# tlangin/MDQTPlasmaSims

Hardware: AMD Instinct MI355X
Metric: particle-steps/sec (MD+QT) at N=3.5k and N=1M; 1/2/4/8-GPU scaling (higher is better)
Workload: dtype f64

## Files before the change

### mdqtplasmasims_amd/csrc/mdqt_engine.cpp

```cpp

#include <math.h>
#include <stdarg.h>
#include <stdlib.h>

#include <algorithm>
#include <thread>

#include "mdqt_ctx.hpp"
#include "mdqt_init_sample.hpp"

using namespace mdqt;

namespace {

thread_local std::string g_err;

struct cx { double re, im; };
inline cx cx_make(double r, double i) { return {r, i}; }
inline cx cx_mul(cx a, cx b) { return {a.re * b.re - a.im * b.im, a.re * b.im + a.im * b.re}; }
inline cx cx_add(cx a, cx b) { return {a.re + b.re, a.im + b.im}; }
inline cx cx_sub(cx a, cx b) { return {a.re - b.re, a.im - b.im}; }
inline cx cx_conj(cx a) { return {a.re, -a.im}; }


// ... 232 lines not shown
        else if (k == 4 || k == 5) e1 = 1.;
        else if (k == 6 || k == 7) e1 = 1. - q.kRat;
        else if (k == 8 || k == 9) e1 = -(1. + q.kRat);
        else if (k >= 10) e1 = q.kRat - 1.;
        f.mi0[k] = -(h * e0);
        f.mi1[k] = -(h * e1);
    }
    f.dms[8] = -(h * q.a8);  f.dmc[8] = h * q.a8;
    f.dms[9] = -(h * q.a11); f.dmc[9] = h * q.a11;
    f.dms[5] = h * q.a8;     f.dmc[5] = h * q.a8;
    f.dms[4] = h * q.a11;    f.dmc[4] = h * q.a11;
    const double kS = q.kickS * q.dtQ * q.gamToE, kD = q.kickD * q.dtQ * q.gamToE;
    struct KW { int row, col, g; double sgn, scale; };
    const KW kws[12] = {{1, 2, 0, 1., kS},  {0, 3, 2, 1., kS},  {1, 4, 4, -1., kS}, {0, 5, 5, -1., kS},
                        {8, 5, 8, 1., kD},  {9, 4, 11, 1., kD}, {10, 3, 14, 1., kD}, {11, 2, 17, 1., kD},
                        {6, 5, 6, -1., kD}, {7, 4, 9, -1., kD}, {8, 3, 12, -1., kD}, {9, 2, 15, -1., kD}};
    for (const KW& w : kws)
        for (int j = 0; j < 3; ++j)
            if (kFastCol[w.col][j] == w.row) f.kw[j][w.col] = -(w.sgn * (w.scale * gs[w.g]));
    f.cphi = 2. * (1. + q.kRat) * q.gamToE;
    if (p->qt_model != 0) build_pump_tables(p, q, f);
    f.dt2 = (0.5 * q.dtQ) * (0.5 * q.dtQ);
    for (int k = 0; k < 4; ++k) q.hdPh[k] = f.hdp[2 + k];
    FastTab& fl = s->ftabL;
    fl = f;
    {
        double kw = 0.;
        for (int j = 0; j < 3; ++j)
            for (int k = 0; k < 16; ++k) kw += fabs(f.kw[j][k]);
        q.kickmax = fmax(fabs(q.vKick), fabs(q.vKickDP)) + 16. * kw;
    }
    q.im01 = 1;
    for (int k = 0; k < 16; ++k)
        if (f.cre[0][k] != 0. || f.cre[1][k] != 0.) q.im01 = 0;
    if (p->qt_model == 0) {
        memset(&fl, 0, sizeof fl);
        fl.cphi = f.cphi; fl.dt2 = f.dt2;
        for (int l = 0; l < 16; ++l) {
            for (int j = 0; j < 3; ++j) fl.col[j][l] = l;
            const int k = state_of_lane0(l);
            if (k >= NS) continue;
            for (int j = 0; j < 3; ++j) {
                fl.cre[j][l] = f.cre[j][k]; fl.cim[j][l] = f.cim[j][k]; fl.kw[j][l] = f.kw[j][k];
            }
            fl.dms[l] = f.dms[k]; fl.dmc[l] = f.dmc[k]; fl.mre[l] = f.mre[k];
            fl.mi0[l] = f.mi0[k]; fl.mi1[l] = f.mi1[k]; fl.hdp[l] = f.hdp[k];
// ... 485 lines not shown
```

### mdqtplasmasims_amd/csrc/mdqt_ensemble_qt.hip

```cpp
#include "mdqt_ens_args.hpp"
#include "mdqt_qtfast.hpp"

namespace mdqt {

#define LANE_ENS_KERNELS(SUFFIX, ATTR, JUNI)                                                                        \
    template <bool DPPX, bool FAST>                                                                                 \
    __global__ __launch_bounds__(256) ATTR void k_substeps_lanes_r_ens##SUFFIX(const SubstepArgs* __restrict__ jobs, \
                                                                               const FastTab* __restrict__ tab) {   \
        const SubstepArgs& a = jobs[blockIdx.y];                                                                    \
        if ((int)blockIdx.x * kLaneIons >= a.n) return;                                                             \
        lane_substeps<DPPX, FAST, false, false, false, false, JUNI>(a, tab, blockIdx.x);                            \
    }                                                                                                               \
    template <bool DPPX, bool EDZ, bool NORN = false>                                                               \
    __global__ __launch_bounds__(256) ATTR void k_substeps_lanes_im_ens##SUFFIX(const SubstepArgs* __restrict__ jobs, \
                                                                                const FastTab* __restrict__ tab) {  \
        const SubstepArgs& a = jobs[blockIdx.y];                                                                    \
        if ((int)blockIdx.x * kLaneIons >= a.n) return;                                                             \
        lane_substeps<DPPX, true, false, true, EDZ, NORN, JUNI>(a, tab, blockIdx.x);                                \
    }
LANE_ENS_KERNELS(, , true)
LANE_ENS_KERNELS(_w3, __attribute__((amdgpu_waves_per_eu(3, 3))), false)
#undef LANE_ENS_KERNELS

hipError_t launch_substeps_r_ens(const SubstepArgs* jobs, const SubstepArgs& a, int njobs, int max_n, const FastTab* tab,
                                 int wpe, hipStream_t s, hipEvent_t ev0, hipEvent_t ev1, int* instance) {
    if (njobs <= 0 || max_n <= 0 || a.nsub <= 0) return hipSuccess;
    if (!jobs || njobs > 65535 || a.nsub > MAXSUB || a.qc.model != 0 || a.arrive || a.U) return hipErrorInvalidValue;
    if (wpe != 0 && wpe != 3) return hipErrorInvalidValue;
    const dim3 gl((max_n + kLaneIons - 1) / kLaneIons, njobs), bl(kLaneWG);
    const FastTab* lt = tab + 1;
    const QTKernel inst = lane_qt_instance(a);
    switch (inst) {
    case QTK_LANES_IM_EDZ:
        if (wpe == 3) launch_timed(k_substeps_lanes_im_ens_w3<true, true, true>, gl, bl, s, ev0, ev1, jobs, lt);
        else launch_timed(k_substeps_lanes_im_ens<true, true, true>, gl, bl, s, ev0, ev1, jobs, lt);
        break;
    case QTK_LANES_IM_EDZ_RN: launch_timed(k_substeps_lanes_im_ens<true, true>, gl, bl, s, ev0, ev1, jobs, lt); break;
    case QTK_LANES_IM: launch_timed(k_substeps_lanes_im_ens<true, false>, gl, bl, s, ev0, ev1, jobs, lt); break;
    case QTK_LANES_R_FAST: launch_timed(k_substeps_lanes_r_ens<true, true>, gl, bl, s, ev0, ev1, jobs, lt); break;
    case QTK_LANES_R: launch_timed(k_substeps_lanes_r_ens<true, false>, gl, bl, s, ev0, ev1, jobs, lt); break;
    default: return hipErrorInvalidValue;
    }
    if (instance) *instance = inst;
    return hipGetLastError();
}

}
```

### mdqtplasmasims_amd/csrc/mdqt_ensemble_sweep_qt.hip

```cpp
#include "mdqt_ens_args.hpp"
#include "mdqt_qtfast.hpp"

namespace mdqt {

#define LANE_SWEEP_KERNELS(SUFFIX, ATTR, JUNI)                                                                         \
    template <bool DPPX, bool FAST>                                                                                    \
    __global__ __launch_bounds__(256) ATTR void k_substeps_lanes_r_sweep##SUFFIX(const SubstepArgs* __restrict__ jobs, \
                                                                                 const FastTab* __restrict__ tabs,     \
                                                                                 const int* __restrict__ point) {      \
        const SubstepArgs& a = jobs[blockIdx.y];                                                                       \
        if ((int)blockIdx.x * kLaneIons >= a.n) return;                                                                \
        lane_substeps<DPPX, FAST, false, false, false, false, JUNI>(a, tabs + point[blockIdx.y], blockIdx.x);          \
    }                                                                                                                  \
    template <bool DPPX, bool EDZ, bool NORN = false>                                                                  \
    __global__ __launch_bounds__(256) ATTR void k_substeps_lanes_im_sweep##SUFFIX(const SubstepArgs* __restrict__ jobs, \
                                                                                  const FastTab* __restrict__ tabs,    \
                                                                                  const int* __restrict__ point) {     \
        const SubstepArgs& a = jobs[blockIdx.y];                                                                       \
        if ((int)blockIdx.x * kLaneIons >= a.n) return;                                                                \
        lane_substeps<DPPX, true, false, true, EDZ, NORN, JUNI>(a, tabs + point[blockIdx.y], blockIdx.x);              \
    }
LANE_SWEEP_KERNELS(, , true)
LANE_SWEEP_KERNELS(_w3, __attribute__((amdgpu_waves_per_eu(3, 3))), false)
#undef LANE_SWEEP_KERNELS

hipError_t launch_substeps_r_sweep(const SubstepArgs* jobs, const SubstepArgs* h, int njobs, int max_n, const FastTab* tabs,
                                   const int* point, int wpe, hipStream_t s, hipEvent_t ev0, hipEvent_t ev1, int* instance,
                                   int* differs) {
    if (differs) *differs = -1;
    if (njobs <= 0 || max_n <= 0) return hipSuccess;
    if (!jobs || !h || !tabs || !point || njobs > 65535) return hipErrorInvalidValue;
    const SubstepArgs& a = h[0];
    if (a.nsub <= 0) return hipSuccess;
    if (a.nsub > MAXSUB || a.qc.model != 0 || a.arrive || a.U) return hipErrorInvalidValue;
    if (wpe != 0 && wpe != 3) return hipErrorInvalidValue;
    for (int k = 1; k < njobs; ++k)
        if (sweep_choice_differs(a, h[k])) {
            if (differs) *differs = k;
            return hipErrorInvalidValue;
        }
    const dim3 gl((max_n + kLaneIons - 1) / kLaneIons, njobs), bl(kLaneWG);
    const QTKernel inst = lane_qt_instance(a);
    switch (inst) {
    case QTK_LANES_IM_EDZ:
        if (wpe == 3) launch_timed(k_substeps_lanes_im_sweep_w3<true, true, true>, gl, bl, s, ev0, ev1, jobs, tabs, point);
        else launch_timed(k_substeps_lanes_im_sweep<true, true, true>, gl, bl, s, ev0, ev1, jobs, tabs, point);
        break;
    case QTK_LANES_IM_EDZ_RN: launch_timed(k_substeps_lanes_im_sweep<true, true>, gl, bl, s, ev0, ev1, jobs, tabs, point); break;
    case QTK_LANES_IM: launch_timed(k_substeps_lanes_im_sweep<true, false>, gl, bl, s, ev0, ev1, jobs, tabs, point); break;
    case QTK_LANES_R_FAST: launch_timed(k_substeps_lanes_r_sweep<true, true>, gl, bl, s, ev0, ev1, jobs, tabs, point); break;
    case QTK_LANES_R: launch_timed(k_substeps_lanes_r_sweep<true, false>, gl, bl, s, ev0, ev1, jobs, tabs, point); break;
    default: return hipErrorInvalidValue;
    }
    if (instance) *instance = inst;
    return hipGetLastError();
}

}
```

### mdqtplasmasims_amd/csrc/mdqt_internal.hpp

```cpp
#pragma once
#include <hip/hip_runtime.h>
#if defined(__HIP__)
#include <hip/hip_ext.h>
#include <type_traits>
#endif
#include <stdint.h>

namespace mdqt {

constexpr int NS = 12;
constexpr int NBINS = 2001;
constexpr int MAXSUB = 32;
constexpr int NSTATIC = 20;
constexpr double kKdeV2 = 1. / (2. * 0.002 * 0.002);
constexpr double kKdeSkip = 0.0773;
static_assert(kKdeV2 * kKdeSkip * kKdeSkip * (1. - 1e-12) >= 746.0, "KDE skip threshold must lie beyond exp's underflow");

constexpr int kStaticRC[NSTATIC][2] = {
    {0, 3}, {0, 5}, {1, 2}, {1, 4}, {2, 1}, {2, 9}, {2, 11}, {3, 0}, {3, 8}, {3, 10},
    {4, 1}, {4, 7}, {5, 0}, {5, 6}, {6, 5}, {7, 4}, {8, 3}, {9, 2}, {10, 3}, {11, 2}};

struct QTConst {
    double dtQ, gamToE;
    double h, dtHalf, invh;
    double pv2q;
    double kRat, r;
    double det, detDP;
    double kickS, kickD;
    double vKick, vKickDP;
    double pD;
    double dP[4];
    double hdP[4];
    double hdPh[4];
    double a8, a11;
    double Mre[NSTATIC], Mim[NSTATIC];
    double thS3, thS4;
    double thD[4][2];
    double gs[18];
    double kickmax;
    int renorm;
    int im01;
    int model;
    uint32_t seed, job;
};

struct LaneTab {
    int colA[16], colB[16], colC[16];
    int order[16], hasB[16], hasC[16];
    int dynB[16], dynC[16];
    double cAre[16], cAim[16], cBre[16], cBim[16], cCre[16], cCim[16];
    double dynScale[16];
    double gA[16], gB[16];
    double dP[16];
    double hd[16];
};

constexpr int NMODELS = 4;
constexpr int kModelStates[NMODELS] = {12, 7, 7, 5};
constexpr int kFastColM[NMODELS][NS][3] = {
    {{5, 12, 3}, {4, 12, 2}, {9, 11, 1}, {8, 10, 0}, {1, 7, 9}, {0, 6, 8},
     {12, 5, 12}, {12, 4, 12}, {3, 12, 5}, {2, 12, 4}, {12, 3, 12}, {12, 2, 12}},
    {{2, 4, 0}, {3, 5, 1}, {0, 2, 2}, {1, 3, 3}, {0, 4, 4}, {1, 5, 5},
     {6, 6, 6}, {7, 7, 7}, {8, 8, 8}, {9, 9, 9}, {10, 10, 10}, {11, 11, 11}},
    {{4, 0, 0}, {5, 1, 1}, {2, 2, 2}, {3, 3, 3}, {0, 4, 4}, {1, 5, 5},
     {6, 6, 6}, {7, 7, 7}, {8, 8, 8}, {9, 9, 9}, {10, 10, 10}, {11, 11, 11}},
    {{3, 0, 0}, {2, 1, 1}, {1, 2, 2}, {0, 3, 3}, {4, 4, 4}, {5, 5, 5},
     {6, 6, 6}, {7, 7, 7}, {8, 8, 8}, {9, 9, 9}, {10, 10, 10}, {11, 11, 11}}};
// ... 127 lines not shown
    else g(std::integral_constant<int, 0>{});
}
#endif

enum QTKernel : int {
    QTK_NONE = 0,
    QTK_LANES_IM_EDZ = 1,
    QTK_LANES_IM = 2,
    QTK_LANES_R_FAST = 3,
    QTK_LANES_R = 4,
    QTK_LANES_R_PUMP_FAST = 5,
    QTK_LANES_R_PUMP = 6,
    QTK_LANES_IM_EDZ_RN = 7,
    QTK_THREAD_R = 10,
    QTK_MD_STEP = 20,
    QTK_EXACT_LANES = 30,
    QTK_EXACT_THREAD = 40,
};
hipError_t launch_substeps(const SubstepArgs& a, const LaneTab* tab, int mode, int fast, hipStream_t s,
                           hipEvent_t ev0 = nullptr, hipEvent_t ev1 = nullptr, int* instance = nullptr);
hipError_t launch_substeps_r(const SubstepArgs& a, const FastTab* tab, int mode, hipStream_t s,
                             hipEvent_t ev0 = nullptr, hipEvent_t ev1 = nullptr,
                             int* instance = nullptr);
hipError_t launch_md_step(const N3Args& f, const SubstepArgs& a, const FastTab* tab, int variant, hipStream_t s,
                          hipEvent_t ev0 = nullptr, hipEvent_t ev1 = nullptr);

hipError_t launch_tag_spin_up(const double* psi, int n, int S, uint64_t gid0, uint64_t q, const QTConst& qc,
                              int* tags, hipStream_t s);
hipError_t launch_sum_vx(const double* V, int n, double* out, hipStream_t s, double* avg = nullptr, int N = 0);
hipError_t launch_output_pack(const double* V, const double* psi, int n, int S, int model, double* out,
                              hipStream_t s);
hipError_t launch_energy_sums(const double* V, int n, int S, const double* vxAvg,
                              const double* urow, double* out, hipStream_t s);
hipError_t launch_kde(const double* V, int n, int S, const double* vxAvg, double* Ppart,
                      int nchunk, double* Pout, hipStream_t s);

}
```

### mdqtplasmasims_amd/csrc/mdqt_options.cpp

```cpp

#include <math.h>
#include <stdlib.h>

#include "mdqt_ctx.hpp"

using namespace mdqt;

struct TierConst { const char *radius, *bound; int mdqt_ctx::*exp; int level; };
static const TierConst kTierConsts[] = {
    {"force_far_radius", "force_far_bound", &mdqt_ctx::far_exp, 1},
    {"force_mid_radius", "force_mid_bound", &mdqt_ctx::mid_exp, 5},
    {"force_vfar_radius", "force_vfar_bound", &mdqt_ctx::vfar_exp, 2},
    {"force_ufar_radius", "force_ufar_bound", &mdqt_ctx::ufar_exp, 3},
};
static double tier_const(const mdqt_ctx* s, int k, int level, double* bound) {
    *bound = 0.;
    const bool on = s->use_n3b && s->sort_mode != 0 && s->force_variant == 1 && !s->guard;
    return on ? tier_radius(s, k, level, bound) : s->L / 2.;
}

extern "C" double mdqt_get_const(const mdqt_ctx* s, const char* n) {
    if (!strcmp(n, "gamToEinsteinFreq")) return s->gamToE;
    if (!strcmp(n, "quantumTimestep")) return s->dtQ;
    if (!strcmp(n, "plasmaToQuantumTimestepRatio")) return s->ratio;
// ... 64 lines not shown
        tier_radii(s, a);
        return error_eps(s, a);
    }
    for (const TierConst& tc : kTierConsts) {
        const bool radius = !strcmp(n, tc.radius);
        if (!radius && strcmp(n, tc.bound)) continue;
        double bound;
        double r = tier_const(s, s->*tc.exp, tc.level, &bound);
        if (tc.level == 3) {
            if (r < s->L / 2. && s->L / 2. > 80. * s->lDeb) { r = s->L / 2.; bound = 0.; }
            double b32 = 0.;
            if (r < s->L / 2.) tier_radius(s, s->ufar_exp, 4, &b32);
            bound += b32;
        }
        return radius ? r : bound;
    }
    if (!strcmp(n, "force_ufar32_radius")) {
        double bound;
        const double r3 = mdqt_get_const(s, "force_ufar_radius");
        return r3 < s->L / 2. ? tier_radius(s, s->ufar_exp, 4, &bound) : s->L / 2.;
    }
    if (!strcmp(n, "fused_step")) return s->fused_opt;
    if (!strcmp(n, "qt_im01")) return s->qc.im01;
    if (!strcmp(n, "potential_n3")) return s->n3_potential;
    if (!strcmp(n, "potential_plan")) return s->pot_plan;
    if (!strcmp(n, "force_n3b_pairs")) return s->n3b_pairs;
    if (!strcmp(n, "md_step_fused")) return s->last_fused;
    if (!strcmp(n, "qt_kernel")) return s->last_qt_kernel;
    if (!strcmp(n, "qt_kernel_nseg")) return s->last_qt_nseg;
    if (!strcmp(n, "force_slots")) return s->nslots;
    if (!strcmp(n, "n3b_blocks")) return s->use_n3b ? s->n3b.Phi - s->n3b.Plo : 0;
    if (!strcmp(n, "n3b_block_count")) return s->use_n3b ? s->n3b.NB : 0;
    if (!strcmp(n, "slab_S")) return s->S;
    if (!strncmp(n, "gs", 2)) return s->gs[atoi(n + 2)];
    return NAN;
}

enum Invalidates {
    NOTHING,
    SETTLE,
    SETTLE_RESET,
    SETTLE_AUX,
};
struct Option {
    const char* name;
    int lo, hi;
// ... 6 lines not shown

static int set_force_scheme(mdqt_ctx* s, int value) {
    if (value == 2 && s->p.world_size != 1) return set_error("force_scheme 2 needs world_size 1");
    if (settle_forces(s)) return -1;
    s->scheme_opt = value;
    choose_segments(s);
    return ensure_aux(s);
}
static int set_expt_force_sig(mdqt_ctx* s, int value) {
    if (value && arrive_setup(s)) return -1;
    s->force_arrive = value ? s->dArrive : nullptr;
    return 0;
}
static int set_qt_im01(mdqt_ctx* s, int value) {
    if (value) {
        int ok = 1;
        for (int k = 0; k < 16; ++k)
            if (s->ftab.cre[0][k] != 0. || s->ftab.cre[1][k] != 0.) ok = 0;
        if (!ok) return set_error("qt_im01: the static coupling slots are not purely imaginary");
    }
    s->qc.im01 = value;
    return 0;
}
static int set_force_balance(mdqt_ctx* s, int value) {
    if (value != s->balance_opt) {
        if (settle_forces(s)) return -1;
        s->balance_opt = value;
        if (s->use_n3b) {
            const int W = s->p.world_size;
            n3b_set_range(s->n3b, (int)((long)s->p.rank * s->n3b.NB / W), (int)((long)(s->p.rank + 1) * s->n3b.NB / W));
            s->balanced = false;
            if (ensure_aux(s)) return -1;
        }
    }
    return 0;
}
static int set_qt_enabled(mdqt_ctx* s, int value) { s->p.qt_enabled = value; return 0; }
static int set_qt_math(mdqt_ctx* s, int value) {
    if (value != 2 && s->p.qt_model != 0) return set_error("the optical-pumping qt_models need qt_math 2");
    s->qt_math = value;
    return 0;
}

static const Option kOptions[] = {
    {"force_scheme", 0, 3, "force_scheme must be 0 (auto), 1 (rows), 2 (Newton-3 tiles) or 3 (Newton-3 blocks)",
     NOTHING, nullptr, set_force_scheme},
    {"expt_force_sig", 0, 1, "expt_force_sig must be 0 or 1", NOTHING, nullptr, set_expt_force_sig},
    {"potential_n3", 0, 1, "potential_n3 must be 0 or 1", NOTHING, &mdqt_ctx::n3_potential},
    {"force_n3b_pairs", 0, 1, "force_n3b_pairs must be 0 (8 waves, one I tile each) or 1 (4 waves, two each)",
     SETTLE, &mdqt_ctx::n3b_pairs},
    {"potential_plan", 0, 1, "potential_plan must be 0 (every pair to L/2) or 1 (the plan)", NOTHING, &mdqt_ctx::pot_plan},
    {"qt_im01", 0, 1, "qt_im01 must be 0 or 1", NOTHING, nullptr, set_qt_im01},
    {"fused_step", 0, 1, "fused_step must be 0 or 1", NOTHING, &mdqt_ctx::fused_opt},
    {"overlap", 0, 1, "overlap must be 0 or 1", NOTHING, &mdqt_ctx::overlap_opt},
    {"force_ufar_exp", 0, 300, "force_ufar_exp must be 0 (off) .. 300", SETTLE_RESET, &mdqt_ctx::ufar_exp, nullptr, form_measured},
    {"force_vfar_exp", 0, 300, "force_vfar_exp must be 0 (off) .. 300", SETTLE_RESET, &mdqt_ctx::vfar_exp, nullptr, form_measured},
    {"force_mid_exp", 0, 300, "force_mid_exp must be 0 (off) .. 300", SETTLE_RESET, &mdqt_ctx::mid_exp, nullptr, form_measured},
    {"force_far_exp", 0, 300, "force_far_exp must be 0 (off) .. 300", SETTLE_RESET, &mdqt_ctx::far_exp, nullptr, form_measured},
    {"force_tail_exp", 0, 300, "force_tail_exp must be 0 (exact) .. 300", SETTLE_RESET, &mdqt_ctx::tail_exp},
    {"force_form_mode", 0, 2, "force_form_mode must be 0 (a priori), 1 (measured) or 2 (measured, sharing an exact tail's eps)",
     SETTLE_RESET, &mdqt_ctx::form_mode},
    {"force_tail_mode", 0, 1, "force_tail_mode must be 0 (a priori) or 1 (measured)", SETTLE_RESET, &mdqt_ctx::tail_mode},
    {"force_balance", 0, 1, "force_balance must be 0 (equal block counts) or 1 (by work)", NOTHING, nullptr, set_force_balance},
    {"force_tile_split", 0, 2, "force_tile_split must be 0 (off), 1 (halves) or 2 (quarters)", SETTLE_AUX, &mdqt_ctx::split_opt},
    {"force_split_cus", 0, 65536, "force_split_cus must be 0 (the device's CU count) or a CU count",
     SETTLE_AUX, &mdqt_ctx::split_cus},
    {"force_reduce_mask", 0, 1, "force_reduce_mask must be 0 (every j-slot) or 1 (the written ones)",
     SETTLE, &mdqt_ctx::tmask_mode},
    {"force_ax1", 0, 1, "force_ax1 must be 0 (off) or 1 (where the skip radius reaches L/2)", SETTLE, &mdqt_ctx::ax1_mode},
    {"force_sort", 0, 2, "force_sort must be 0 (off), 1 (on) or 2 (sorted, no skipping)", SETTLE_AUX, &mdqt_ctx::sort_mode},
    {"qt_enabled", 0, 1, "qt_enabled must be 0 or 1", NOTHING, nullptr, set_qt_enabled},
    {"qt_math", 0, 2, "qt_math must be 0 (exact), 1 (FMA-contracted) or 2 (reassociated)", NOTHING, nullptr, set_qt_math},
    {"force_kernel", 0, 1, "force_kernel must be 0 (exact) or 1 (fast)", SETTLE_RESET, &mdqt_ctx::force_variant},
    {"init_threads", 0, 256, "init_threads must be in [0, 256]", NOTHING, &mdqt_ctx::init_threads},
    {"substep_kernel", 0, 2, "substep_kernel must be 0 (auto), 1 (thread/ion) or 2 (lanes/ion)", NOTHING, &mdqt_ctx::substep_mode},
// ... 127 lines not shown
```

### mdqtplasmasims_amd/csrc/mdqt_qtfast.hip

```cpp
#include "mdqt_qtfast.hpp"
#include "mdqt_pump_device.hpp"

namespace mdqt {

template <int MODEL>
__device__ __forceinline__ double sum_p(const double* Tp) {
    if constexpr (MODEL == 0) return ((Tp[0] + Tp[2]) + Tp[1]) + Tp[3];
    return (Tp[0] + Tp[1]) + (Tp[2] + Tp[3]);
}
template <int MODEL>
__device__ __forceinline__ double tree_lanes(const double* vs) {
    double v[16];
#pragma unroll
    for (int l = 0; l < 16; ++l) {
        const int st = MODEL == 0 ? state_of_lane0(l) : l;
        v[l] = st < NS ? vs[st] : 0.;
    }
    return tree16n(v);
}

template <int MODEL>
__global__ __launch_bounds__(256) void k_substeps_r(SubstepArgs a, const FastTab* __restrict__ tab) {
    constexpr const int(&COL)[NS][3] = kFastColM[MODEL];
    const int i = blockIdx.x * 256 + threadIdx.x;
// ... 181 lines not shown
    } else {
        if (variant == 1) launch_timed(k_md_step<false, 1>, gl, bl, s, ev0, ev1, f, a, lt);
        else launch_timed(k_md_step<false, 0>, gl, bl, s, ev0, ev1, f, a, lt);
    }
    return hipGetLastError();
}

#if defined(MDQT_EXPT_QTSTAMPS)
extern "C" int mdqt_expt_qt_stamps(unsigned long long* out, int nwaves) {
    return hipMemcpyFromSymbol(out, HIP_SYMBOL(g_qt_stamps), sizeof(unsigned long long) * 16 * nwaves) == hipSuccess ? 0 : -1;
}
#endif

hipError_t launch_substeps_r(const SubstepArgs& a, const FastTab* tab, int mode, hipStream_t s, hipEvent_t ev0,
                             hipEvent_t ev1, int* instance) {
    if (a.n <= 0 || a.nsub <= 0) return hipSuccess;
    if (a.nsub > MAXSUB) return hipErrorInvalidValue;
    if (mode == 0) mode = (a.n < kLaneKernelMaxIons) ? 2 : 1;
    if (a.qc.model < 0 || a.qc.model >= NMODELS) return hipErrorInvalidValue;
    const dim3 gl((a.n + kLaneIons - 1) / kLaneIons), bl(kLaneWG), gt((a.n + 255) / 256), b(256);
    int inst = QTK_THREAD_R + a.qc.model;
    if (mode == 2) {
        const FastTab* lt = tab + 1;
        switch (inst = lane_qt_instance(a)) {
        case QTK_LANES_IM_EDZ: launch_timed(k_substeps_lanes_im<true, true, true>, gl, bl, s, ev0, ev1, a, lt); break;
        case QTK_LANES_IM_EDZ_RN: launch_timed(k_substeps_lanes_im<true, true>, gl, bl, s, ev0, ev1, a, lt); break;
        case QTK_LANES_IM: launch_timed(k_substeps_lanes_im<true, false>, gl, bl, s, ev0, ev1, a, lt); break;
        case QTK_LANES_R_FAST: launch_timed(k_substeps_lanes_r<true, true>, gl, bl, s, ev0, ev1, a, lt); break;
        case QTK_LANES_R: launch_timed(k_substeps_lanes_r<true, false>, gl, bl, s, ev0, ev1, a, lt); break;
        case QTK_LANES_R_PUMP_FAST: launch_timed(k_substeps_lanes_r<false, true>, gl, bl, s, ev0, ev1, a, lt); break;
        case QTK_LANES_R_PUMP: launch_timed(k_substeps_lanes_r<false, false>, gl, bl, s, ev0, ev1, a, lt); break;
        default: return hipErrorInvalidValue;
        }
    }
    else if (a.qc.model == 0) launch_timed(k_substeps_r<0>, gt, b, s, ev0, ev1, a, tab);
    else if (a.qc.model == 1) launch_timed(k_substeps_r<1>, gt, b, s, ev0, ev1, a, tab);
    else if (a.qc.model == 2) launch_timed(k_substeps_r<2>, gt, b, s, ev0, ev1, a, tab);
    else launch_timed(k_substeps_r<3>, gt, b, s, ev0, ev1, a, tab);
    if (instance) *instance = inst;
    return hipGetLastError();
}

__global__ __launch_bounds__(256) void k_tag_spin_up(const double* __restrict__ psi, int n, int S, uint64_t gid0,
                                                     uint64_t q, QTConst qc, int* __restrict__ tags) {
    const int i = blockIdx.x * 256 + threadIdx.x;
    if (i >= n) return;
    tag_spin_up_ion(psi, i, S, gid0, q, qc, tags);
// ... 11 lines not shown
```

### mdqtplasmasims_amd/csrc/mdqt_qtfast.hpp

```cpp
#pragma once
#include "mdqt_internal.hpp"
#if defined(__HIP__)
#include "mdqt_device.hpp"
#include "mdqt_pairs.hpp"

#include <math.h>

#include <type_traits>

namespace mdqt {

constexpr int kLaneWG = 256;
static_assert(kLaneWG % 64 == 0 && kLaneWG >= 128, "whole waves; the first 128 threads stage the sincos table");
constexpr int kRows = 4;
constexpr int kLaneIons = kLaneWG / 64 * kRows;

__device__ __forceinline__ double rsq_nr(double x) { return rsq3(x); }
__device__ __forceinline__ double nrm2(cxd y) { return fma(y.re, y.re, y.im * y.im); }
__device__ __forceinline__ double rho_im_r(cxd a, cxd b) { return fma(a.im, b.re, -(a.re * b.im)); }

__device__ __forceinline__ cxd row_r(cxd md, cxd y, cxd c0, cxd y0, cxd c1, cxd y1, cxd c2, cxd y2) {
    double re = md.re * y.re, im = md.re * y.im;
    re = fma(-md.im, y.im, re);  im = fma(md.im, y.re, im);
    re = fma(c0.re, y0.re, re);  im = fma(c0.re, y0.im, im);
// ... 120 lines not shown
    double a = dpp<BCAST(0)>(T);
    a = fmac_bcast<3>(a, T, one);
    a = fmac_bcast<4>(a, T, one);
    return fmac_bcast<7>(a, T, one);
}

__device__ __forceinline__ void qt_store(double* p, double v) {
    __hip_atomic_store(p, v, __ATOMIC_RELAXED, __HIP_MEMORY_SCOPE_AGENT);
}

#if defined(MDQT_EXPT_QTSTAMPS)
__device__ unsigned long long g_qt_stamps[16 * 4096];
#define QT_STAMP(slot, v) (st_[slot] = (v))
#define QT_JCOUNT(c) (st_[7] += (__builtin_amdgcn_ballot_w64(c) != 0))
#else
#define QT_STAMP(slot, v) ((void)0)
#define QT_JCOUNT(c) ((void)0)
#endif

#if defined(MDQT_EXPT_MDSTAMPS)
__device__ unsigned long long g_md_stamps[4 * 4096];
#endif

template <bool DPPX, bool FAST, bool FUSED, bool IM01 = false, bool EDZ = false, bool NORN = false, bool JUNI = !FUSED>
__device__ __forceinline__ void lane_substeps(const SubstepArgs& a, const FastTab* __restrict__ tab, int blk) {
#if defined(MDQT_EXPT_QTSTAMPS)
    unsigned long long st_[16] = {};
#endif
    QT_STAMP(0, __builtin_amdgcn_s_memtime());
    QT_STAMP(4, __builtin_amdgcn_s_memrealtime());
    const int k = threadIdx.x & 15;
    const int grp = threadIdx.x >> 4;
    const int iraw = blk * (kLaneWG / 16) + grp;
    const bool store = iraw < a.n;
    const int i = store ? iraw : a.n - 1;
    const QTConst& qc = a.qc;
    const int S = a.S;
    const int st = DPPX ? state_of_lane0(k) : k;
    const int cy = DPPX ? 9 : 12, cz = DPPX ? 10 : 13;
    const int c = (k == cy) ? 1 : (k == cz) ? 2 : 0;
    const bool owner = (k == 0) || (k == cy) || (k == cz);
    const int base = threadIdx.x & ~15;
    const int l0 = base + tab->col[0][k], l1 = base + tab->col[1][k], l2 = base + tab->col[2][k];
    const cxd c0 = {tab->cre[0][k], tab->cim[0][k]}, c1 = {tab->cre[1][k], tab->cim[1][k]};
    const double c2re = tab->cre[2][k], c2im = tab->cim[2][k], dms = tab->dms[k], dmc = tab->dmc[k];
    const double mre = tab->mre[k], mi0 = tab->mi0[k], mi1 = tab->mi1[k], hdp = tab->hdp[k];
    const double kw0 = tab->kw[0][k], kw1 = tab->kw[1][k], kw2 = tab->kw[2][k];
    const double cphi = tab->cphi, DT2 = tab->dt2;
// ... 38 lines not shown
            slot_add(t);
        }
    };
    double t0[4][3];
    if (FAST) {
        if (!FUSED) slot_round(k, t0, false);
    } else if (nseg > 1) {
        if (!a.arrive) slot_partials(false);
    } else {
        f = a.F[(size_t)c * S + i];
    }
    QT_STAMP(9, __builtin_amdgcn_s_memtime());
    const double L = a.L, dt = qc.dtQ, DT = 0.5 * dt;
    double dtq_v = qc.dtQ, pv2q_v = qc.pv2q;
    asm volatile("" : "+v"(dtq_v), "+v"(pv2q_v));
    const uint64_t gid = a.gid0 + (uint64_t)i;
    const uint32_t movmask = a.movmask;
    __shared__ double edt[MAXSUB];
    const double edv = (threadIdx.x < MAXSUB && a.expdet_zero == 0 && (int)threadIdx.x < a.nsub)
                           ? a.expDet[threadIdx.x] : 0.;
    __shared__ double sct[128];
    const double sctv = threadIdx.x < 128 ? kSinCos64[threadIdx.x] : 0.;
    __shared__ double su[kLaneWG / 16][MAXSUB][2];
    if (FAST || a.do_qt) {
        if (a.U) {
            if (k == 0) { su[grp][0][0] = a.U[i]; su[grp][0][1] = a.U[(size_t)S + i]; }
        } else {
            for (int s = k; s < a.nsub; s += 16) {
                double x0, x1;
                philox_pair(qc, gid, a.q0 + (uint64_t)s, 0, x0, x1);
                su[grp][s][0] = x0;
                su[grp][s][1] = x1;
            }
        }
    }
    QT_STAMP(8, __builtin_amdgcn_s_memtime());
    if (!FAST && a.arrive) {
        if (threadIdx.x == 0) {
            int it = 0;
            const unsigned long long* cnt = a.arrive + (blk * (kLaneWG / 16)) / 64;
            while (__hip_atomic_load(cnt, __ATOMIC_ACQUIRE, __HIP_MEMORY_SCOPE_AGENT) < a.arrive_target) {
                for (int z = 0; z < a.arrive_sleep; ++z) __builtin_amdgcn_s_sleep(1);
                if (++it > (1 << 21)) { *a.spin_err = 1; break; }
            }
        }
        __syncthreads();
        __atomic_thread_fence(__ATOMIC_ACQUIRE);
        if (nseg > 1) slot_partials(true);
    }
// ... 9 lines not shown
        __syncthreads();
        __atomic_thread_fence(__ATOMIC_ACQUIRE);
#if defined(MDQT_EXPT_MDSTAMPS)
        if (threadIdx.x == 0 && blockIdx.x < 4096) g_md_stamps[4 * blockIdx.x + 2] = __builtin_amdgcn_s_memrealtime();
#endif
        slot_round(k, t0, true);
    }
    if (FAST) {
        slot_add(t0);
        for (int s0 = k + 64; s0 < nseg; s0 += 64) {
            double t[4][3];
            slot_round(s0, t, FUSED);
            slot_add(t);
        }
    }
    QT_STAMP(6, __builtin_amdgcn_s_memtime());
    if (FAST || nseg > 1) {
        const double fx = lane_tree16(qf[0]), fy = lane_tree16(qf[1]), fz = lane_tree16(qf[2]);
        f = c == 0 ? fx : c == 1 ? fy : fz;
        if (store && owner) qt_store(&a.F[(size_t)c * S + i], f);
    }
    if (threadIdx.x < MAXSUB) edt[threadIdx.x] = edv;
    if (threadIdx.x < 128) sct[threadIdx.x] = sctv;
    __syncthreads();
    __shared__ double2 xg[DPPX ? 1 : kLaneWG];
    auto exchange = [&](cxd y, cxd& y0, cxd& y1, cxd& y2) {
        if constexpr (DPPX) {
            y0 = {dpp<QP_XOR2>(y.re), dpp<QP_XOR2>(y.im)};
            y1 = {dpp<ROR(8)>(y.re), dpp<ROR(8)>(y.im)};
            y2 = {dpp<QP_XOR1>(y.re), dpp<QP_XOR1>(y.im)};
            return;
        }
        wave_sync();
        xg[threadIdx.x] = make_double2(y.re, y.im);
        wave_sync();
        const double2 t0 = xg[l0], t1 = xg[l1], t2 = xg[l2];
        y0 = {t0.x, t0.y}; y1 = {t1.x, t1.y}; y2 = {t2.x, t2.y};
    };
    auto drift = [&](double& pp, double& vv, int sub) {
        const bool moving = FAST || ((movmask >> sub) & 1u);
        pp = half_drift(pp, vv, f, moving, DT, DT2, L);
        vv = vv + dt * f;
        pp = half_drift(pp, vv, f, moving, DT, DT2, L);
    };
    QT_STAMP(1, __builtin_amdgcn_s_memtime());
    if (!FAST && !a.do_qt) {
// ... 87 lines not shown
                    (void)dummy;
                } else {
                    double x0, x1;
                    philox_pair(qc, gid, a.q0 + (uint64_t)s, k < 8 ? 1 : 2, x0, x1);
                    randDOrS = dpp<BCAST(0)>(x0);
                    randDir = dpp<BCAST(0)>(x1);
                    rand3 = dpp<BCAST(8)>(x0);
                }
                return (DPPX || qc.model == 0)
                           ? jump_target(qc, n3, n4, n5, n6, u2, randDOrS, randDir, rand3, jkick)
                           : jump_target_pump(qc, n3, n4, n5, n6, u2, randDOrS, randDir, rand3, jkick);
            };
            if constexpr (JUNI) {
            auto jump_substep = [&](auto tape) {
                const double kick_rk = rk_kick();
                const cxd w_rk = rk_stages();
                double kick_j;
                const int target = jump(tape, kick_j);
                w = {nojump ? w_rk.re : (st == target ? 1. : 0.), nojump ? w_rk.im : 0.};
                kick = nojump ? kick_rk : kick_j;
                tPart = nojump ? tPart : 0.;
                next_phase();
            };
            if (__builtin_expect(__builtin_amdgcn_ballot_w64(!nojump) == 0, 1)) {
                kick = rk_kick();
                next_phase();
                w = rk_stages();
            } else if (a.U) {
                jump_substep(std::true_type{});
            } else {
                jump_substep(std::false_type{});
            }
            } else if (nojump) {
                kick = rk_kick();
                next_phase();
                w = rk_stages();
            } else {
                tPart = 0;
                int target;
                if (a.U) target = jump(std::true_type{}, kick);
                else target = jump(std::false_type{}, kick);
                w = {st == target ? 1. : 0., 0.};
                next_phase();
            }
            if constexpr (decltype(chk)::value)
                if (!(fabs(phin) < 1048576.)) sincos(phin, &snn, &csn);
            if (!NORN && qc.renorm) w = [&] {
                const double r = rsq_nr(lane_norm16(nrm2(w), one));
                return cxd{w.re * r, w.im * r};
            }();
            v = vn;
            p = pn;
            u = un;
            sn = snn;
// ... 49 lines not shown

namespace mdqt {

inline QTKernel lane_qt_instance(const SubstepArgs& a) {
    const uint64_t all = (1ull << a.nsub) - 1;
    const bool allmove = a.do_step && a.do_qt && a.nseg >= 1 && !a.arrive && (a.movmask & all) == all;
    if (a.qc.model != 0) return allmove ? QTK_LANES_R_PUMP_FAST : QTK_LANES_R_PUMP;
    if (!allmove) return QTK_LANES_R;
    if (!a.qc.im01) return QTK_LANES_R_FAST;
    if (!a.expdet_zero) return QTK_LANES_IM;
    return a.qc.renorm ? QTK_LANES_IM_EDZ_RN : QTK_LANES_IM_EDZ;
}
inline const char* sweep_choice_differs(const SubstepArgs& a, const SubstepArgs& b) {
    if (a.nsub != b.nsub) return "nsub";
    if (a.do_step != b.do_step) return "do_step";
    if (a.do_qt != b.do_qt) return "do_qt";
    if (a.movmask != b.movmask) return "movmask (t > 0 per substep)";
    if (a.expdet_zero != b.expdet_zero) return "expdet_zero (fracOfSig == 0 against != 0)";
    if (a.qc.im01 != b.qc.im01) return "qt_im01";
    if (a.qc.renorm != b.qc.renorm) return "reNormalizewvFns";
    if (a.qc.model != b.qc.model) return "qt_model";
    if ((a.nseg >= 1) != (b.nseg >= 1)) return "nseg";
    if (!a.arrive != !b.arrive || !a.U != !b.U) return "arrive / U (another launch scheme)";
    return nullptr;
}

}
```

Measured before the change: 2.886 billion.

## Stage jump constants in LDS and optionally predraw jump random candidates

```diff
diff --git a/mdqtplasmasims_amd/csrc/mdqt_engine.cpp b/mdqtplasmasims_amd/csrc/mdqt_engine.cpp
--- a/mdqtplasmasims_amd/csrc/mdqt_engine.cpp
+++ b/mdqtplasmasims_amd/csrc/mdqt_engine.cpp
@@ -278,6 +278,7 @@
     if (p->qt_model != 0) build_pump_tables(p, q, f);
     f.dt2 = (0.5 * q.dtQ) * (0.5 * q.dtQ);
     for (int k = 0; k < 4; ++k) q.hdPh[k] = f.hdp[2 + k];
+    jump_predraw_setup(q, f.hdp, 1);
     FastTab& fl = s->ftabL;
     fl = f;
     {
diff --git a/mdqtplasmasims_amd/csrc/mdqt_ensemble_qt.hip b/mdqtplasmasims_amd/csrc/mdqt_ensemble_qt.hip
--- a/mdqtplasmasims_amd/csrc/mdqt_ensemble_qt.hip
+++ b/mdqtplasmasims_amd/csrc/mdqt_ensemble_qt.hip
@@ -3,23 +3,24 @@
 
 namespace mdqt {
 
-#define LANE_ENS_KERNELS(SUFFIX, ATTR, JUNI)                                                                        \
+#define LANE_ENS_KERNELS(SUFFIX, ATTR, JUNI, JPRE)                                                                    \
     template <bool DPPX, bool FAST>                                                                                 \
     __global__ __launch_bounds__(256) ATTR void k_substeps_lanes_r_ens##SUFFIX(const SubstepArgs* __restrict__ jobs, \
                                                                                const FastTab* __restrict__ tab) {   \
         const SubstepArgs& a = jobs[blockIdx.y];                                                                    \
         if ((int)blockIdx.x * kLaneIons >= a.n) return;                                                             \
-        lane_substeps<DPPX, FAST, false, false, false, false, JUNI>(a, tab, blockIdx.x);                            \
+        lane_substeps<DPPX, FAST, false, false, false, false, JUNI, JPRE>(a, tab, blockIdx.x);                            \
     }                                                                                                               \
     template <bool DPPX, bool EDZ, bool NORN = false>                                                               \
     __global__ __launch_bounds__(256) ATTR void k_substeps_lanes_im_ens##SUFFIX(const SubstepArgs* __restrict__ jobs, \
                                                                                 const FastTab* __restrict__ tab) {  \
         const SubstepArgs& a = jobs[blockIdx.y];                                                                    \
         if ((int)blockIdx.x * kLaneIons >= a.n) return;                                                             \
-        lane_substeps<DPPX, true, false, true, EDZ, NORN, JUNI>(a, tab, blockIdx.x);                                \
+        lane_substeps<DPPX, true, false, true, EDZ, NORN, JUNI, JPRE>(a, tab, blockIdx.x);                                \
     }
-LANE_ENS_KERNELS(, , true)
-LANE_ENS_KERNELS(_w3, __attribute__((amdgpu_waves_per_eu(3, 3))), false)
+LANE_ENS_KERNELS(, , true, true)
+LANE_ENS_KERNELS(_jp0, , true, false)
+LANE_ENS_KERNELS(_w3, __attribute__((amdgpu_waves_per_eu(3, 3))), false, false)
 #undef LANE_ENS_KERNELS
 
 hipError_t launch_substeps_r_ens(const SubstepArgs* jobs, const SubstepArgs& a, int njobs, int max_n, const FastTab* tab,
@@ -30,15 +31,16 @@
     const dim3 gl((max_n + kLaneIons - 1) / kLaneIons, njobs), bl(kLaneWG);
     const FastTab* lt = tab + 1;
     const QTKernel inst = lane_qt_instance(a);
+    auto go = [&](auto k_pre, auto k_jp0) { launch_timed(a.qc.jpre ? k_pre : k_jp0, gl, bl, s, ev0, ev1, jobs, lt); };
     switch (inst) {
     case QTK_LANES_IM_EDZ:
         if (wpe == 3) launch_timed(k_substeps_lanes_im_ens_w3<true, true, true>, gl, bl, s, ev0, ev1, jobs, lt);
-        else launch_timed(k_substeps_lanes_im_ens<true, true, true>, gl, bl, s, ev0, ev1, jobs, lt);
+        else go(k_substeps_lanes_im_ens<true, true, true>, k_substeps_lanes_im_ens_jp0<true, true, true>);
         break;
-    case QTK_LANES_IM_EDZ_RN: launch_timed(k_substeps_lanes_im_ens<true, true>, gl, bl, s, ev0, ev1, jobs, lt); break;
-    case QTK_LANES_IM: launch_timed(k_substeps_lanes_im_ens<true, false>, gl, bl, s, ev0, ev1, jobs, lt); break;
-    case QTK_LANES_R_FAST: launch_timed(k_substeps_lanes_r_ens<true, true>, gl, bl, s, ev0, ev1, jobs, lt); break;
-    case QTK_LANES_R: launch_timed(k_substeps_lanes_r_ens<true, false>, gl, bl, s, ev0, ev1, jobs, lt); break;
+    case QTK_LANES_IM_EDZ_RN: go(k_substeps_lanes_im_ens<true, true>, k_substeps_lanes_im_ens_jp0<true, true>); break;
+    case QTK_LANES_IM: go(k_substeps_lanes_im_ens<true, false>, k_substeps_lanes_im_ens_jp0<true, false>); break;
+    case QTK_LANES_R_FAST: go(k_substeps_lanes_r_ens<true, true>, k_substeps_lanes_r_ens_jp0<true, true>); break;
+    case QTK_LANES_R: go(k_substeps_lanes_r_ens<true, false>, k_substeps_lanes_r_ens_jp0<true, false>); break;
     default: return hipErrorInvalidValue;
     }
     if (instance) *instance = inst;
diff --git a/mdqtplasmasims_amd/csrc/mdqt_ensemble_sweep_qt.hip b/mdqtplasmasims_amd/csrc/mdqt_ensemble_sweep_qt.hip
--- a/mdqtplasmasims_amd/csrc/mdqt_ensemble_sweep_qt.hip
+++ b/mdqtplasmasims_amd/csrc/mdqt_ensemble_sweep_qt.hip
@@ -3,14 +3,14 @@
 
 namespace mdqt {
 
-#define LANE_SWEEP_KERNELS(SUFFIX, ATTR, JUNI)                                                                         \
+#define LANE_SWEEP_KERNELS(SUFFIX, ATTR, JUNI, JPRE)                                                                     \
     template <bool DPPX, bool FAST>                                                                                    \
     __global__ __launch_bounds__(256) ATTR void k_substeps_lanes_r_sweep##SUFFIX(const SubstepArgs* __restrict__ jobs, \
                                                                                  const FastTab* __restrict__ tabs,     \
                                                                                  const int* __restrict__ point) {      \
         const SubstepArgs& a = jobs[blockIdx.y];                                                                       \
         if ((int)blockIdx.x * kLaneIons >= a.n) return;                                                                \
-        lane_substeps<DPPX, FAST, false, false, false, false, JUNI>(a, tabs + point[blockIdx.y], blockIdx.x);          \
+        lane_substeps<DPPX, FAST, false, false, false, false, JUNI, JPRE>(a, tabs + point[blockIdx.y], blockIdx.x);          \
     }                                                                                                                  \
     template <bool DPPX, bool EDZ, bool NORN = false>                                                                  \
     __global__ __launch_bounds__(256) ATTR void k_substeps_lanes_im_sweep##SUFFIX(const SubstepArgs* __restrict__ jobs, \
@@ -18,10 +18,11 @@
                                                                                   const int* __restrict__ point) {     \
         const SubstepArgs& a = jobs[blockIdx.y];                                                                       \
         if ((int)blockIdx.x * kLaneIons >= a.n) return;                                                                \
-        lane_substeps<DPPX, true, false, true, EDZ, NORN, JUNI>(a, tabs + point[blockIdx.y], blockIdx.x);              \
+        lane_substeps<DPPX, true, false, true, EDZ, NORN, JUNI, JPRE>(a, tabs + point[blockIdx.y], blockIdx.x);              \
     }
-LANE_SWEEP_KERNELS(, , true)
-LANE_SWEEP_KERNELS(_w3, __attribute__((amdgpu_waves_per_eu(3, 3))), false)
+LANE_SWEEP_KERNELS(, , true, true)
+LANE_SWEEP_KERNELS(_jp0, , true, false)
+LANE_SWEEP_KERNELS(_w3, __attribute__((amdgpu_waves_per_eu(3, 3))), false, false)
 #undef LANE_SWEEP_KERNELS
 
 hipError_t launch_substeps_r_sweep(const SubstepArgs* jobs, const SubstepArgs* h, int njobs, int max_n, const FastTab* tabs,
@@ -41,15 +42,16 @@
         }
     const dim3 gl((max_n + kLaneIons - 1) / kLaneIons, njobs), bl(kLaneWG);
     const QTKernel inst = lane_qt_instance(a);
+    auto go = [&](auto k_pre, auto k_jp0) { launch_timed(a.qc.jpre ? k_pre : k_jp0, gl, bl, s, ev0, ev1, jobs, tabs, point); };
     switch (inst) {
     case QTK_LANES_IM_EDZ:
         if (wpe == 3) launch_timed(k_substeps_lanes_im_sweep_w3<true, true, true>, gl, bl, s, ev0, ev1, jobs, tabs, point);
-        else launch_timed(k_substeps_lanes_im_sweep<true, true, true>, gl, bl, s, ev0, ev1, jobs, tabs, point);
+        else go(k_substeps_lanes_im_sweep<true, true, true>, k_substeps_lanes_im_sweep_jp0<true, true, true>);
         break;
-    case QTK_LANES_IM_EDZ_RN: launch_timed(k_substeps_lanes_im_sweep<true, true>, gl, bl, s, ev0, ev1, jobs, tabs, point); break;
-    case QTK_LANES_IM: launch_timed(k_substeps_lanes_im_sweep<true, false>, gl, bl, s, ev0, ev1, jobs, tabs, point); break;
-    case QTK_LANES_R_FAST: launch_timed(k_substeps_lanes_r_sweep<true, true>, gl, bl, s, ev0, ev1, jobs, tabs, point); break;
-    case QTK_LANES_R: launch_timed(k_substeps_lanes_r_sweep<true, false>, gl, bl, s, ev0, ev1, jobs, tabs, point); break;
+    case QTK_LANES_IM_EDZ_RN: go(k_substeps_lanes_im_sweep<true, true>, k_substeps_lanes_im_sweep_jp0<true, true>); break;
+    case QTK_LANES_IM: go(k_substeps_lanes_im_sweep<true, false>, k_substeps_lanes_im_sweep_jp0<true, false>); break;
+    case QTK_LANES_R_FAST: go(k_substeps_lanes_r_sweep<true, true>, k_substeps_lanes_r_sweep_jp0<true, true>); break;
+    case QTK_LANES_R: go(k_substeps_lanes_r_sweep<true, false>, k_substeps_lanes_r_sweep_jp0<true, false>); break;
     default: return hipErrorInvalidValue;
     }
     if (instance) *instance = inst;
diff --git a/mdqtplasmasims_amd/csrc/mdqt_internal.hpp b/mdqtplasmasims_amd/csrc/mdqt_internal.hpp
--- a/mdqtplasmasims_amd/csrc/mdqt_internal.hpp
+++ b/mdqtplasmasims_amd/csrc/mdqt_internal.hpp
@@ -12,6 +12,7 @@
 constexpr int NBINS = 2001;
 constexpr int MAXSUB = 32;
 constexpr int NSTATIC = 20;
+constexpr int kJumpRow = 16;
 constexpr double kKdeV2 = 1. / (2. * 0.002 * 0.002);
 constexpr double kKdeSkip = 0.0773;
 static_assert(kKdeV2 * kKdeSkip * kKdeSkip * (1. - 1e-12) >= 746.0, "KDE skip threshold must lie beyond exp's underflow");
@@ -42,7 +43,21 @@
     int im01;
     int model;
     uint32_t seed, job;
-};
+    int jpre;
+    double dpcand;
+    double jrow[kJumpRow];
+};
+enum JumpRow { JR_PD = 0, JR_VKICK = 1, JR_VKICKDP = 2, JR_THS3 = 3, JR_THS4 = 4, JR_Q0 = 5, JR_THD = 8 };
+inline void jump_predraw_setup(QTConst& q, const double* hdp16, int mode) {
+    double m = 0.;
+    for (int k = 0; k < 16; ++k) m = hdp16[k] > m ? hdp16[k] : m;
+    q.jpre = mode;
+    q.dpcand = mode == 2 ? 2. * m : mode == 3 ? 2. : -1.;
+    for (double& x : q.jrow) x = 0.;
+    q.jrow[JR_PD] = q.pD; q.jrow[JR_VKICK] = q.vKick; q.jrow[JR_VKICKDP] = q.vKickDP;
+    q.jrow[JR_THS3] = q.thS3; q.jrow[JR_THS4] = q.thS4;
+    for (int r = 0; r < 4; ++r) { q.jrow[JR_THD + 2 * r] = q.thD[r][0]; q.jrow[JR_THD + 2 * r + 1] = q.thD[r][1]; }
+}
 
 struct LaneTab {
     int colA[16], colB[16], colC[16];
@@ -216,6 +231,8 @@
 hipError_t launch_substeps_r(const SubstepArgs& a, const FastTab* tab, int mode, hipStream_t s,
                              hipEvent_t ev0 = nullptr, hipEvent_t ev1 = nullptr,
                              int* instance = nullptr);
+hipError_t launch_substeps_lanes_jp0(const SubstepArgs& a, const FastTab* lt, QTKernel inst, dim3 gl, dim3 bl,
+                                     hipStream_t s, hipEvent_t ev0, hipEvent_t ev1);
 hipError_t launch_md_step(const N3Args& f, const SubstepArgs& a, const FastTab* tab, int variant, hipStream_t s,
                           hipEvent_t ev0 = nullptr, hipEvent_t ev1 = nullptr);
 
diff --git a/mdqtplasmasims_amd/csrc/mdqt_options.cpp b/mdqtplasmasims_amd/csrc/mdqt_options.cpp
--- a/mdqtplasmasims_amd/csrc/mdqt_options.cpp
+++ b/mdqtplasmasims_amd/csrc/mdqt_options.cpp
@@ -110,6 +110,8 @@
     }
     if (!strcmp(n, "fused_step")) return s->fused_opt;
     if (!strcmp(n, "qt_im01")) return s->qc.im01;
+    if (!strcmp(n, "qt_jump_predraw")) return s->qc.jpre;
+    if (!strcmp(n, "qt_jump_candidate_dp")) return s->qc.dpcand;
     if (!strcmp(n, "potential_n3")) return s->n3_potential;
     if (!strcmp(n, "potential_plan")) return s->pot_plan;
     if (!strcmp(n, "force_n3b_pairs")) return s->n3b_pairs;
@@ -162,6 +164,10 @@
     s->qc.im01 = value;
     return 0;
 }
+static int set_qt_jump_predraw(mdqt_ctx* s, int value) {
+    jump_predraw_setup(s->qc, s->ftab.hdp, value);
+    return 0;
+}
 static int set_force_balance(mdqt_ctx* s, int value) {
     if (value != s->balance_opt) {
         if (settle_forces(s)) return -1;
@@ -191,6 +197,8 @@
      SETTLE, &mdqt_ctx::n3b_pairs},
     {"potential_plan", 0, 1, "potential_plan must be 0 (every pair to L/2) or 1 (the plan)", NOTHING, &mdqt_ctx::pot_plan},
     {"qt_im01", 0, 1, "qt_im01 must be 0 or 1", NOTHING, nullptr, set_qt_im01},
+    {"qt_jump_predraw", 0, 3, "qt_jump_predraw must be 0 (earlier block), 1 (LDS constants), 2 (candidates predrawn) or 3 (every substep)",
+     NOTHING, nullptr, set_qt_jump_predraw},
     {"fused_step", 0, 1, "fused_step must be 0 or 1", NOTHING, &mdqt_ctx::fused_opt},
     {"overlap", 0, 1, "overlap must be 0 or 1", NOTHING, &mdqt_ctx::overlap_opt},
     {"force_ufar_exp", 0, 300, "force_ufar_exp must be 0 (off) .. 300", SETTLE_RESET, &mdqt_ctx::ufar_exp, nullptr, form_measured},
diff --git a/mdqtplasmasims_amd/csrc/mdqt_qtfast.hip b/mdqtplasmasims_amd/csrc/mdqt_qtfast.hip
--- a/mdqtplasmasims_amd/csrc/mdqt_qtfast.hip
+++ b/mdqtplasmasims_amd/csrc/mdqt_qtfast.hip
@@ -227,7 +227,11 @@
     int inst = QTK_THREAD_R + a.qc.model;
     if (mode == 2) {
         const FastTab* lt = tab + 1;
-        switch (inst = lane_qt_instance(a)) {
+        inst = lane_qt_instance(a);
+        if (a.qc.model == 0 && !a.qc.jpre) {
+            const hipError_t e = launch_substeps_lanes_jp0(a, lt, (QTKernel)inst, gl, bl, s, ev0, ev1);
+            if (e != hipSuccess) return e;
+        } else switch (inst) {
         case QTK_LANES_IM_EDZ: launch_timed(k_substeps_lanes_im<true, true, true>, gl, bl, s, ev0, ev1, a, lt); break;
         case QTK_LANES_IM_EDZ_RN: launch_timed(k_substeps_lanes_im<true, true>, gl, bl, s, ev0, ev1, a, lt); break;
         case QTK_LANES_IM: launch_timed(k_substeps_lanes_im<true, false>, gl, bl, s, ev0, ev1, a, lt); break;
diff --git a/mdqtplasmasims_amd/csrc/mdqt_qtfast.hpp b/mdqtplasmasims_amd/csrc/mdqt_qtfast.hpp
--- a/mdqtplasmasims_amd/csrc/mdqt_qtfast.hpp
+++ b/mdqtplasmasims_amd/csrc/mdqt_qtfast.hpp
@@ -166,8 +166,10 @@
 __device__ unsigned long long g_md_stamps[4 * 4096];
 #endif
 
-template <bool DPPX, bool FAST, bool FUSED, bool IM01 = false, bool EDZ = false, bool NORN = false, bool JUNI = !FUSED>
+template <bool DPPX, bool FAST, bool FUSED, bool IM01 = false, bool EDZ = false, bool NORN = false, bool JUNI = !FUSED,
+          bool JPRE = JUNI && DPPX>
 __device__ __forceinline__ void lane_substeps(const SubstepArgs& a, const FastTab* __restrict__ tab, int blk) {
+    static_assert(!JPRE || (JUNI && DPPX), "JPRE: the wave-uniform jump block of the model-0 layout");
 #if defined(MDQT_EXPT_QTSTAMPS)
     unsigned long long st_[16] = {};
 #endif
@@ -252,9 +254,48 @@
     __shared__ double sct[128];
     const double sctv = threadIdx.x < 128 ? kSinCos64[threadIdx.x] : 0.;
     __shared__ double su[kLaneWG / 16][MAXSUB][2];
+    constexpr int kJumpSlots = 8;
+    __shared__ __attribute__((aligned(16))) double jrow[JPRE ? kJumpRow : 1];
+    __shared__ uint32_t jcand[JPRE ? kLaneWG / 16 : 1];
+    __shared__ double jdraw[JPRE ? kLaneWG / 16 : 1][3][kJumpSlots];
+    double jrv = 0.;
+    if constexpr (JPRE)
+        if (threadIdx.x < kJumpRow)
+            jrv = threadIdx.x == JR_Q0 ? __longlong_as_double((long long)a.q0) : qc.jrow[threadIdx.x];
     if (FAST || a.do_qt) {
         if (a.U) {
             if (k == 0) { su[grp][0][0] = a.U[i]; su[grp][0][1] = a.U[(size_t)S + i]; }
+        } else if constexpr (JPRE) {
+            uint32_t cand = 0;
+            const bool predraw = qc.dpcand >= 0.;
+            for (int s0 = 0; s0 < a.nsub; s0 += 16) {
+                const int s = s0 + k;
+                double x0 = 2., x1;
+                if (s < a.nsub) {
+                    philox_pair(qc, gid, a.q0 + (uint64_t)s, 0, x0, x1);
+                    su[grp][s][0] = x0;
+                    su[grp][s][1] = x1;
+                }
+                if (predraw) {
+                    const uint64_t b = __builtin_amdgcn_ballot_w64(x0 < qc.dpcand);
+                    cand |= ((uint32_t)(b >> (threadIdx.x & 48)) & 0xFFFFu) << s0;
+                }
+            }
+            if (k == 0) jcand[grp] = cand;
+            uint32_t m = cand;
+            const int cs = k & 7;
+#pragma unroll
+            for (int j = 0; j < kJumpSlots - 1; ++j) m = j < cs ? m & (m - 1) : m;
+            if (predraw && m) {
+                double x0, x1;
+                philox_pair(qc, gid, a.q0 + (uint64_t)__builtin_ctz(m), k < 8 ? 1 : 2, x0, x1);
+                if (k < 8) {
+                    jdraw[grp][0][cs] = x0;
+                    jdraw[grp][1][cs] = x1;
+                } else {
+                    jdraw[grp][2][cs] = x0;
+                }
+            }
         } else {
             for (int s = k; s < a.nsub; s += 16) {
                 double x0, x1;
@@ -310,6 +351,8 @@
     }
     if (threadIdx.x < MAXSUB) edt[threadIdx.x] = edv;
     if (threadIdx.x < 128) sct[threadIdx.x] = sctv;
+    if constexpr (JPRE)
+        if (threadIdx.x < kJumpRow) jrow[threadIdx.x] = jrv;
     __syncthreads();
     __shared__ double2 xg[DPPX ? 1 : kLaneWG];
     auto exchange = [&](cxd y, cxd& y0, cxd& y1, cxd& y2) {
@@ -443,6 +486,53 @@
                 tPart = nojump ? tPart : 0.;
                 next_phase();
             };
+            auto jump_substep_pre = [&](auto) {
+                const double kick_rk = rk_kick();
+                const double nk = sq(w);
+                const double n3 = dpp<BCAST(0)>(nk), n4 = dpp<BCAST(4)>(nk), n5 = dpp<BCAST(3)>(nk), n6 = dpp<BCAST(7)>(nk);
+                int jr0 = 0;
+                asm volatile("" : "+v"(jr0));
+                const double* jr = jrow + jr0;
+                const uint32_t cand = jcand[grp];
+                const int slot = __builtin_popcount(cand & ((1u << s) - 1u));
+                const bool hit = ((cand >> s) & 1u) != 0 && slot < kJumpSlots;
+                double randDOrS, randDir, rand3;
+                if (__builtin_amdgcn_ballot_w64(!nojump && !hit) == 0) {
+                    const int sl = slot & (kJumpSlots - 1);
+                    randDOrS = jdraw[grp][0][sl];
+                    randDir = jdraw[grp][1][sl];
+                    rand3 = jdraw[grp][2][sl];
+                } else {
+                    double x0, x1;
+                    const uint64_t q0 = (uint64_t)__double_as_longlong(jr[JR_Q0]);
+                    philox_pair(qc, gid, q0 + (uint64_t)s, k < 8 ? 1 : 2, x0, x1);
+                    randDOrS = dpp<BCAST(0)>(x0);
+                    randDir = dpp<BCAST(0)>(x1);
+                    rand3 = dpp<BCAST(8)>(x0);
+                }
+                double pD = jr[JR_PD], vKick = jr[JR_VKICK], vKickDP = jr[JR_VKICKDP];
+                asm volatile("" : "+v"(pD), "+v"(vKick), "+v"(vKickDP));
+                const bool sDecay = !(randDOrS < pD);
+                const double kmag = sDecay ? vKick : vKickDP;
+                kick = nojump ? kick_rk : (randDir < 0.5) ? kmag : -kmag;
+                tPart = nojump ? tPart : 0.;
+                next_phase();
+                const cxd w_rk = rk_stages();
+                const double tot = n3 + n4 + n5 + n6;
+                const double pk = nk / tot;
+                const double prob3 = dpp<BCAST(0)>(pk), prob4 = dpp<BCAST(4)>(pk), prob5 = dpp<BCAST(3)>(pk);
+                const int ge3 = !(u2 < prob3), ge34 = ge3 & !(u2 < prob3 + prob4);
+                const int ge345 = ge34 & !(u2 < prob3 + prob4 + prob5);
+                const int row = ge3 + ge34 + ge345;
+                double2 th = *reinterpret_cast<const double2*>(&jr[JR_THD + 2 * row]);
+                double thS3 = jr[JR_THS3], thS4 = jr[JR_THS4];
+                asm volatile("" : "+v"(th.x), "+v"(th.y), "+v"(thS3), "+v"(thS4));
+                const int d0 = rand3 < th.x, d1 = rand3 < th.y;
+                const int tD = 9 - row + d0 + (d0 | d1);
+                const int tS = (row == 0) | ((row == 1) & !(rand3 < thS3)) | ((row == 2) & (rand3 < thS4));
+                const int target = sDecay ? tS : tD;
+                w = {nojump ? w_rk.re : (st == target ? 1. : 0.), nojump ? w_rk.im : 0.};
+            };
             if (__builtin_expect(__builtin_amdgcn_ballot_w64(!nojump) == 0, 1)) {
                 kick = rk_kick();
                 next_phase();
@@ -450,7 +540,8 @@
             } else if (a.U) {
                 jump_substep(std::true_type{});
             } else {
-                jump_substep(std::false_type{});
+                if constexpr (JPRE) jump_substep_pre(0);
+                else jump_substep(std::false_type{});
             }
             } else if (nojump) {
                 kick = rk_kick();
@@ -546,6 +637,7 @@
     if (a.qc.model != b.qc.model) return "qt_model";
     if ((a.nseg >= 1) != (b.nseg >= 1)) return "nseg";
     if (!a.arrive != !b.arrive || !a.U != !b.U) return "arrive / U (another launch scheme)";
+    if (!a.qc.jpre != !b.qc.jpre) return "qt_jump_predraw (0 against != 0)";
     return nullptr;
 }
 
diff --git a/mdqtplasmasims_amd/csrc/mdqt_qtfast_jp0.hip b/mdqtplasmasims_amd/csrc/mdqt_qtfast_jp0.hip
--- /dev/null
+++ b/mdqtplasmasims_amd/csrc/mdqt_qtfast_jp0.hip
@@ -0,0 +1,27 @@
+#include "mdqt_qtfast.hpp"
+
+namespace mdqt {
+
+template <bool FAST>
+__global__ __launch_bounds__(256) void k_substeps_lanes_r_jp0(SubstepArgs a, const FastTab* __restrict__ tab) {
+    lane_substeps<true, FAST, false, false, false, false, true, false>(a, tab, blockIdx.x);
+}
+template <bool EDZ, bool NORN = false>
+__global__ __launch_bounds__(256) void k_substeps_lanes_im_jp0(SubstepArgs a, const FastTab* __restrict__ tab) {
+    lane_substeps<true, true, false, true, EDZ, NORN, true, false>(a, tab, blockIdx.x);
+}
+
+hipError_t launch_substeps_lanes_jp0(const SubstepArgs& a, const FastTab* lt, QTKernel inst, dim3 gl, dim3 bl,
+                                     hipStream_t s, hipEvent_t ev0, hipEvent_t ev1) {
+    switch (inst) {
+    case QTK_LANES_IM_EDZ: launch_timed(k_substeps_lanes_im_jp0<true, true>, gl, bl, s, ev0, ev1, a, lt); break;
+    case QTK_LANES_IM_EDZ_RN: launch_timed(k_substeps_lanes_im_jp0<true>, gl, bl, s, ev0, ev1, a, lt); break;
+    case QTK_LANES_IM: launch_timed(k_substeps_lanes_im_jp0<false>, gl, bl, s, ev0, ev1, a, lt); break;
+    case QTK_LANES_R_FAST: launch_timed(k_substeps_lanes_r_jp0<true>, gl, bl, s, ev0, ev1, a, lt); break;
+    case QTK_LANES_R: launch_timed(k_substeps_lanes_r_jp0<false>, gl, bl, s, ev0, ev1, a, lt); break;
+    default: return hipErrorInvalidValue;
+    }
+    return hipGetLastError();
+}
+
+}
```

New measurement: 2.790 billion. 3.3% lower.
